# bartelvdh/Navtex

Measured on NVIDIA B200. Metric: iq_msamples_per_s, higher is better.
Workload: dtype f32

## Files before the change

navtex_b200/csrc/demod.cu:

```cuda
#include "demod.cuh"

#include <math.h>
#include <stdlib.h>

namespace nvx {

namespace {

constexpr int kThreads = 128;
constexpr int kPer = 3;
constexpr int kTile = kThreads * kPer;

enum { DS_INIT = 0, DS_WAIT = 1, DS_PENDING = 2 };
enum { BY_WAIT = 1, BY_GOT_DX = 2, BY_GOT_RX = 3 };

__constant__ unsigned char c_ltrs[128];
__constant__ unsigned char c_figs[128];
__constant__ float c_tone_r[5];
__constant__ float c_tone_i[5];
__constant__ double c_tone_rd[5];
__constant__ double c_tone_id[5];

struct Emit {
    uint8_t* ev; int* ev_n; int ev_cap; int n;
    bool writer;
    const unsigned char *ltrs, *figs;
// ... 74 lines not shown
__device__ __forceinline__ void fsm_bit_phasing(FsmState& s, bool is_y) {
    if (s.holdoff != 0) { s.holdoff--; return; }
    constexpr unsigned kYmask = (0xFu << 6) | (0x3u << 12) | (0xFu << 20) | (0x3u << 26);
    if (s.match == 29) {
        if (!is_y) { s.enabled = 1; s.nbits = 0; s.shift = 0; s.holdoff = 1100; }
        s.match = 0;
    } else if ((((kYmask >> s.match) & 1u) != 0) == is_y) {
        s.match++;
    } else if (s.match != 6) {
        s.match = 0;
    }
}


__device__ __forceinline__ size_t pitch_y(int p_max) { return (size_t)kHistY + p_max; }
__device__ __forceinline__ size_t pitch_c(int p_max) { return (size_t)kHistC + p_max + kPadC; }
__host__ __device__ __forceinline__ size_t pitch_p(int p_max) { return ((size_t)p_max / kSpb + 2 + 15) & ~(size_t)15; }
__host__ __device__ __forceinline__ size_t pitch_b(int p_max) { return ((size_t)p_max / (kSpb - 1) + 2 + 15) & ~(size_t)15; }

__device__ __forceinline__ double angle_of(float2 cur, float2 prev) {
    const double yi = cur.x, yq = cur.y, pi = prev.x, pq = prev.y;
    const double re = __dadd_rn(__dmul_rn(yi, pi), __dmul_rn(yq, pq));
    const double im = __dsub_rn(__dmul_rn(yq, pi), __dmul_rn(yi, pq));
    return atan2(im, re);
}

__global__ void __launch_bounds__(kThreads) angle_corr_kernel(const DemodArgs a) {
    __shared__ double s_ang[kTile + 8];
    const int ch = blockIdx.y, tile0 = blockIdx.x * kTile, t = threadIdx.x;
    float2* ybuf = a.b.y3 + (size_t)ch * pitch_y(a.b.p_max);
    const float2* y = ybuf + kHistY;
    if (blockIdx.x == 0) {
        const float2* yp = a.y3_prev + (size_t)ch * pitch_y(a.b.p_max) + a.n_prev;
        if (t < kHistY) ybuf[t] = yp[t];
        double* c = a.b.corr + (size_t)ch * pitch_c(a.b.p_max);
        const double* cp = a.corr_prev + (size_t)ch * pitch_c(a.b.p_max) + a.n_prev;
        for (int k = t; k < kHistC; k += kThreads) c[k] = cp[k];
        __syncthreads();
    }
#pragma unroll
    for (int u = 0; u < kPer; ++u) {
        const int m = tile0 + t + u * kThreads;
        if (m < a.n_new) s_ang[8 + t + u * kThreads] = angle_of(y[m], y[m - 1]);
    }
    if (t < 8) s_ang[t] = angle_of(y[tile0 - 8 + t], y[tile0 - 9 + t]);
    __syncthreads();
    double* corr = a.b.corr + (size_t)ch * pitch_c(a.b.p_max) + kHistC;
#pragma unroll
    for (int u = 0; u < kPer; ++u) {
        const int i = t + u * kThreads, m = tile0 + i;
        if (m >= a.n_new) break;
        double c = s_ang[i + 1];
        c = __dadd_rn(c, s_ang[i + 2]);
        c = __dadd_rn(c, s_ang[i + 3]);
        c = __dsub_rn(c, s_ang[i + 5]);
        c = __dsub_rn(c, s_ang[i + 6]);
        c = __dsub_rn(c, s_ang[i + 7]);
        corr[m] = fabs(c);
    }
}

__device__ __forceinline__ bool window_is_y(const float2* __restrict__ y, float* sums) {
    double br = 0.0, bi = 0.0, yr = 0.0, yi = 0.0;
#pragma unroll
    for (int k = 0; k < 5; ++k) {
        const float srf = y[k].x;
        const double si = (double)y[k].y;
        const float fr = c_tone_r[k], fi = c_tone_i[k];
        const double pr = (double)__fmul_rn(srf, fr), pim = (double)__fmul_rn(srf, fi);
        const double qi = __dmul_rn(si, c_tone_id[k]), qr = __dmul_rn(si, c_tone_rd[k]);
        yr = (double)(float)__dadd_rn(yr, __dsub_rn(pr, qi));
        yi = (double)(float)__dadd_rn(yi, __dadd_rn(pim, qr));
        br = (double)(float)__dadd_rn(br, __dadd_rn(pr, qi));
        bi = (double)(float)__dadd_rn(bi, __dsub_rn(qr, pim));
    }
    const float brf = (float)br, bif = (float)bi, yrf = (float)yr, yif = (float)yi;
    if (sums) { sums[0] = brf; sums[1] = bif; sums[2] = yrf; sums[3] = yif; }
    const float eb = __fadd_rn(__fmul_rn(brf, brf), __fmul_rn(bif, bif));
    const float ey = __fadd_rn(__fmul_rn(yrf, yrf), __fmul_rn(yif, yif));
    return !(eb > ey);
}

constexpr int kSumWarps = 4;
constexpr int kGroup = 7;
__global__ void __launch_bounds__(kSumWarps * 32) offset_sum_kernel(const DemodArgs a, int k_lo, int n_rev) {
    __shared__ double s_os[kSumWarps][3][kGroup][kSpb];
    const int warp = threadIdx.x >> 5, lane = threadIdx.x & 31;
    const int kk = lane / kSpb, j = lane - kk * kSpb;
    const long long unit = ((long long)blockIdx.x * kSumWarps + warp) * 3 + kk;
    const bool mine = kk < 3 && unit < (long long)a.channels * n_rev;
    const int ch = mine ? (int)(unit / n_rev) : 0;
    const int K = k_lo + (mine ? (int)(unit % n_rev) : 0);
    const int m_first = (int)(16 + (long long)kCorrLen * K + j - a.seen);
    const double* cur = a.b.corr + (size_t)ch * pitch_c(a.b.p_max) + kHistC + (m_first - 8);
    const double* prev = cur - kCorrLen;
    const int kk2 = lane / kGroup, u2 = lane - kk2 * kGroup;
    const long long unit2 = ((long long)blockIdx.x * kSumWarps + warp) * 3 + kk2;
    const bool judge = kk2 < 3 && unit2 < (long long)a.channels * n_rev;
    const int ch2 = judge ? (int)(unit2 / n_rev) : 0;
    const int w_first = (int)(24 + (long long)kCorrLen * (k_lo + (judge ? (int)(unit2 % n_rev) : 0)) - a.seen);
    uint8_t* picks2 = a.b.picks + (size_t)ch2 * pitch_p(a.b.p_max);

    double run = 0.0;
#pragma unroll 1
    for (int g = 0; g < kCorrLen / kSpb / kGroup; ++g) {
        const int r0 = g * kGroup;
        const int m0 = m_first + kSpb * r0;
        double acc[kGroup];
        if (mine && m0 < a.n_new) {
#pragma unroll
            for (int u = 0; u < kGroup; ++u) {
                run = __dadd_rn(run, __ldg(cur + kSpb * (r0 + u)));
                acc[u] = run;
            }
        } else {
#pragma unroll
            for (int u = 0; u < kGroup; ++u) acc[u] = 0.0;
        }
        if (mine && m0 < a.n_new && m0 + kSpb * (kGroup - 1) >= -8) {
            const double* p = prev + kSpb * (r0 + 1);
            double v[kGroup - 1];
#pragma unroll
            for (int t = 0; t < kGroup - 1; ++t) v[t] = __ldg(p + kSpb * t);
#pragma unroll
            for (int u = 0; u < kGroup - 1; ++u) {
#pragma unroll
                for (int t = u; t < kGroup - 1; ++t) acc[u] = __dadd_rn(acc[u], v[t]);
            }
            p += kSpb * (kGroup - 1);
            const int rest = kCorrLen / kSpb - kGroup - r0;
#pragma unroll 1
            for (int i = 0; i < rest; i += kGroup, p += kSpb * kGroup) {
                double x[kGroup];
#pragma unroll
                for (int t = 0; t < kGroup; ++t) x[t] = __ldg(p + kSpb * t);
#pragma unroll
                for (int t = 0; t < kGroup; ++t) {
#pragma unroll
                    for (int u = 0; u < kGroup; ++u) acc[u] = __dadd_rn(acc[u], x[t]);
                }
            }
        }
        if (kk < 3) {
#pragma unroll
            for (int u = 0; u < kGroup; ++u) {
                const int m = m0 + kSpb * u;
                const bool ok = mine && m < a.n_new && a.seen + m >= kCorrLen + 7;
                s_os[warp][kk][u][j] = ok ? acc[u] : 0.0;
            }
        }
        __syncwarp();
        if (judge) {
            const int w = w_first + kSpb * (r0 + u2);
            if (w >= 0 && w < a.n_new && a.seen + w >= kCorrLen + 15) {
                double best = -1.0;
                int pick = 0;
#pragma unroll
                for (int i = 0; i < kSpb; ++i) {
                    const double x = s_os[warp][kk2][u2][i];
                    if (x > best) { best = x; pick = i; }
                }
                picks2[w / kSpb] = (uint8_t)pick;
            }
        }
        __syncwarp();
    }
}

constexpr int kSeqWarps = 16;
constexpr int kSeqChunk = 256;
constexpr int kSeqPitch = kSeqChunk + 4;
constexpr int kSeqSmem = kSeqWarps * 32 * kSeqPitch;

__device__ __forceinline__ void stage_rows(uint8_t* s_rows, const uint8_t* src, size_t pitch, int ch0, int channels,
                                           int c0, int count, int lane) {
    __syncwarp();
    const int words = (count + 3) >> 2;
    for (int r = 0; r < 32 && ch0 + r < channels; ++r) {
        const uint32_t* g = reinterpret_cast<const uint32_t*>(src + (size_t)(ch0 + r) * pitch + c0);
        uint32_t* d = reinterpret_cast<uint32_t*>(s_rows + r * kSeqPitch);
// ... 155 lines not shown

__global__ void init_state_kernel(ClockState* clock, FsmState* fsm, int channels) {
    const int ch = blockIdx.x * blockDim.x + threadIdx.x;
    if (ch >= channels) return;
    ClockState c = {};
    c.last_pick = -1;
    c.dstate = DS_INIT;
    clock[ch] = c;
    FsmState s = {};
    s.byte_state = BY_WAIT;
    fsm[ch] = s;
}

}

int demod_launches_per_block() { return 5; }
size_t demod_pick_pitch(int p_max) { return pitch_p(p_max); }
size_t demod_bit_pitch(int p_max) { return pitch_b(p_max); }
int demod_reserved_sms(int channels) {
    const int ctas = (channels + kSeqWarps * 32 - 1) / (kSeqWarps * 32);
    return ctas < 4 ? ctas : 4;
}

cudaError_t demod_init_state(const DemodBuffers& b, int channels, cudaStream_t stream) {
    {
        static const struct { unsigned char code; char l, f; } codes[] = {
            {0x07, 'p', 'p'}, {0x0b, 'J', 'b'}, {0x0d, 'W', '2'}, {0x0e, 'A', '-'}, {0x13, 'F', '*'},
            {0x15, 'Y', '6'}, {0x16, 'S', '\''}, {0x19, '-', '-'}, {0x1a, 'D', '%'}, {0x1c, 'Z', '+'},
            {0x1d, '_', ' '}, {0x23, 'C', ':'}, {0x25, 'P', '0'}, {0x26, 'I', '8'}, {0x29, 'G', '*'},
            {0x2a, 'R', '4'}, {0x2c, 'L', ')'}, {0x31, 'M', '.'}, {0x32, 'N', ','}, {0x34, 'H', '*'},
            {0x38, 'O', '9'}, {0x43, 'K', '('}, {0x45, 'Q', '1'}, {0x46, 'U', '7'}, {0x49, 'f', 'f'},
// ... 10 lines not shown
            tr[i] = cosf(ang);
            ti[i] = sinf(ang);
        }
        cudaError_t e;
        if ((e = cudaMemcpyToSymbol(c_ltrs, ltrs, sizeof ltrs)) != cudaSuccess) return e;
        if ((e = cudaMemcpyToSymbol(c_figs, figs, sizeof figs)) != cudaSuccess) return e;
        if ((e = cudaMemcpyToSymbol(c_tone_r, tr, sizeof tr)) != cudaSuccess) return e;
        if ((e = cudaMemcpyToSymbol(c_tone_i, ti, sizeof ti)) != cudaSuccess) return e;
        double trd[5], tid[5];
        for (int i = 0; i < 5; ++i) { trd[i] = tr[i]; tid[i] = ti[i]; }
        if ((e = cudaMemcpyToSymbol(c_tone_rd, trd, sizeof trd)) != cudaSuccess) return e;
        if ((e = cudaMemcpyToSymbol(c_tone_id, tid, sizeof tid)) != cudaSuccess) return e;
    }
    cudaError_t e;
    if ((e = cudaMemsetAsync(b.y3, 0, sizeof(float2) * (size_t)channels * (kHistY + b.p_max), stream)) != cudaSuccess) return e;
    if ((e = cudaMemsetAsync(b.corr, 0, sizeof(double) * (size_t)channels * (kHistC + b.p_max + kPadC), stream)) != cudaSuccess) return e;
    if ((e = cudaMemsetAsync(b.picks, 0, (size_t)channels * pitch_p(b.p_max), stream)) != cudaSuccess) return e;
    init_state_kernel<<<(channels + 127) / 128, 128, 0, stream>>>(b.clock, b.fsm, channels);
    return cudaGetLastError();
}

cudaError_t demod_launch(const DemodArgs& a, cudaStream_t s_ff, cudaStream_t s_seq, cudaEvent_t ff_done, cudaEvent_t* marks) {
    if (a.n_new <= 0 || a.channels <= 0) return cudaSuccess;
    auto mark = [&](int k, cudaStream_t st) { if (marks) cudaEventRecord(marks[k], st); };
    mark(0, s_ff);
    angle_corr_kernel<<<dim3((a.n_new + kTile - 1) / kTile, a.channels), kThreads, 0, s_ff>>>(a);
    mark(1, s_ff);
    {
        const long long lo = a.seen - 8 - (kCorrLen + 15), hi = a.seen + a.n_new - 17;
        const int k_lo = lo <= 0 ? 0 : (int)((lo + kCorrLen - 1) / kCorrLen);
        if (hi >= 0 && (int)(hi / kCorrLen) >= k_lo) {
            const int n_rev = (int)(hi / kCorrLen) - k_lo + 1;
            const long long units = (long long)a.channels * n_rev;
            offset_sum_kernel<<<(unsigned)((units + 3 * kSumWarps - 1) / (3 * kSumWarps)), kSumWarps * 32, 0, s_ff>>>(a, k_lo, n_rev);
        }
    }
    mark(2, s_ff);
    mark(3, s_ff);
    {
        cudaError_t e = cudaEventRecord(ff_done, s_ff);
        if (e != cudaSuccess) return e;
        if (s_seq != s_ff && (e = cudaStreamWaitEvent(s_seq, ff_done, 0)) != cudaSuccess) return e;
    }
    {
        cudaError_t e = cudaFuncSetAttribute(symbol_clock_kernel, cudaFuncAttributeMaxDynamicSharedMemorySize, kSeqSmem);
        if (e == cudaSuccess) e = cudaFuncSetAttribute(fsm_kernel, cudaFuncAttributeMaxDynamicSharedMemorySize, kSeqSmem);
        if (e != cudaSuccess) return e;
    }
    const unsigned seq_ctas = (a.channels + kSeqWarps * 32 - 1) / (kSeqWarps * 32);
    mark(4, s_seq);
// ... 11 lines not shown
```

navtex_b200/csrc/demod.cuh:

```cuda
#pragma once
#include <cuda_runtime.h>
#include <stdint.h>

namespace nvx {

constexpr int kSpb = 9;
constexpr int kCorrLen = 63 * kSpb;
constexpr int kEvAbort = 0x18;

constexpr int kHistY = 16;
constexpr int kHistC = 640;
constexpr int kPadC = 64;

struct ClockState {
    int last_pick;
    int dstate, offs, next_offs, cur, pend;
};

struct FsmState {
    int match;
    int byte_state, figures, nbits, shift;
    unsigned dx_ring;
    int dx_at, dx_full;
    unsigned err_mask;
    int err_at, err_full, err_count;
    int eoe_count, prev_dx_alpha, holdoff, enabled;
};

struct DemodBuffers {
    float2* y3;
    double* corr;
    uint8_t* picks;
    int* bitpos;
    uint8_t* bitval;
    int* nbits;
    ClockState* clock;
    FsmState* fsm;
    int p_max;
};

struct DemodArgs {
    DemodBuffers b;
    const float2* y3_prev;
    const double* corr_prev;
    int n_prev;
    int n_new;
    int channels;
    long long seen;
    uint8_t* events;
    int* ev_count;
    int ev_cap;
    char* bits;
    float* disc;
    int* bit_count;
    int bit_cap;
};

size_t demod_pick_pitch(int p_max);
size_t demod_bit_pitch(int p_max);
int demod_reserved_sms(int channels);
cudaError_t demod_launch(const DemodArgs& a, cudaStream_t s_ff, cudaStream_t s_seq, cudaEvent_t ff_done, cudaEvent_t* marks = nullptr);
cudaError_t demod_init_state(const DemodBuffers& b, int channels, cudaStream_t stream);
int demod_launches_per_block();

}
```

navtex_b200/csrc/engine.cu:

```cuda
#include <cuda.h>
#include <cuda_runtime.h>
#include <math.h>
#include <stdarg.h>
#include <stdio.h>
#include <stdlib.h>
#include <string.h>

#include <condition_variable>
#include <mutex>
#include <string>
#include <thread>
#include <vector>

#include "../../include/navtex_b200.h"
#include "demod.cuh"
#include "fir_cascade.cuh"
#include "fir_long.cuh"
#include "message_assembler.h"

namespace nvx {
int cascade_box_elems(SampleFmt f);
int cascade_tap_class(int n1, int n2, int n3);
int cascade_warm_super(int tap_class);
void cascade_fill_taps(int tap_class, const double* h1, int n1, const double* h2, int n2, const double* h3, int n3, CascadeTaps* out);
// ... 70 lines not shown
    const unsigned w[4] = {(unsigned)v.x, (unsigned)v.y, (unsigned)v.z, (unsigned)v.w};
    int o[8];
#pragma unroll
    for (int k = 0; k < 4; ++k) {
        o[2 * k] = (int)(((w[k] & 0xFFu) - 128u) & 0xFFFFu) | (int)(((((w[k] >> 8) & 0xFFu) - 128u) & 0xFFFFu) << 16);
        o[2 * k + 1] = (int)((((w[k] >> 16) & 0xFFu) - 128u) & 0xFFFFu) | (int)((((w[k] >> 24) - 128u) & 0xFFFFu) << 16);
    }
    int4* dst = reinterpret_cast<int4*>(out + i);
    dst[0] = make_int4(o[0], o[1], o[2], o[3]);
    dst[1] = make_int4(o[4], o[5], o[6], o[7]);
}

}

constexpr int kBuf = 3;

struct nvx_engine {
    nvx_config cfg;
    int S = 0, P_max = 0, channels = 0;
    int C = 2;
    cudaStream_t stream = nullptr;
    cudaStream_t stream_demod = nullptr;
    float2* y3buf[kBuf] = {};
    uint8_t* pickbuf[kBuf] = {};
    cudaEvent_t casc_done[kBuf] = {}, demod_done[kBuf] = {}, ff_done[kBuf] = {};
    long long blocks = 0;
    int last_buf = 0;
    int tap_class = 0;
    int halo = 1960;
    void* tail[nvx::kSampleFmts][2] = {};
    CUtensorMap map_tail[nvx::kSampleFmts][2];
    int tail_cur = 0;
    int fmt = -1;
    short2* u8_wide = nullptr;
    nvx::DemodBuffers db = {};
    double* corrbuf[2] = {nullptr, nullptr};
    uint8_t* d_events[kBuf] = {}; int* d_ev_count[kBuf] = {}; int ev_cap = 0;
    char* d_bits = nullptr; float* d_disc = nullptr; int* d_bit_count = nullptr; int bit_cap = 0;
    uint8_t* h_events[kBuf] = {}; int* h_ev_count[kBuf] = {};
    cudaStream_t stream_copy = nullptr;
    void* stage[2] = {nullptr, nullptr};
    size_t stage_bytes[2] = {0, 0};
    cudaEvent_t copy_done[2] = {}, stage_free[2] = {};
    long long host_pushes = 0;
    long long sb_abs = 0;
    int last_P = 0;
    bool custom_taps = false;
    nvx::CascadeTaps taps;
    nvx::NcoParam* d_nco = nullptr;
    nvx::NcoChan* d_nco_ch = nullptr;
    bool long_taps = false;
    nvx::LongStage lst[3];
    float2* lhist[3][2] = {};
    float2 *y1buf = nullptr, *y2buf = nullptr;
    int lcur = 0;
    nvx::LongTcStage* ltc[2] = {nullptr, nullptr};
    bool mix_on_load = false;
    bool ltc_wanted[2] = {false, false};
    nvx::LongStageTaps ltaps[3];
    std::vector<int> stream_tag;
    bool serial = false;
    bool ff_on_main = true;
    int target_warps[nvx::kSampleFmts] = {576, 576, 576};
    nvx::MessageAssembler assembler;
    std::vector<nvx::AssembledMessage> ready, handed;
    std::vector<nvx_message> view;
    nvx_message_cb cb = nullptr; void* cb_user = nullptr;
    std::thread worker;
    std::mutex mu;
    std::condition_variable cv;
    long long queued = 0, drained = 0;
    long long delivered = 0;
    bool stop = false;
    int worker_rc = 0;
    int timing = 0;
    std::vector<cudaEvent_t> ev_pool;
    struct Span { int a, b, kind; };
    std::vector<Span> spans;
    size_t ev_used = 0;
    std::vector<float> cascade_spans_ms;
    nvx_stats stats = {};
};

namespace {

int free_engine(nvx_engine* e) {
    if (!e) return 0;
    cudaSetDevice(e->cfg.device);
    if (e->stream) cudaStreamSynchronize(e->stream);
    if (e->stream_demod) cudaStreamSynchronize(e->stream_demod);
    if (e->worker.joinable()) {
        {
            std::lock_guard<std::mutex> lk(e->mu);
            e->stop = true;
        }
        e->cv.notify_all();
        e->worker.join();
    }
    for (cudaEvent_t ev : e->ev_pool) cudaEventDestroy(ev);
    for (int f = 0; f < nvx::kSampleFmts; ++f) { cudaFree(e->tail[f][0]); cudaFree(e->tail[f][1]); }
    cudaFree(e->u8_wide);
    cudaFree(e->corrbuf[0]); cudaFree(e->corrbuf[1]); cudaFree(e->db.clock); cudaFree(e->db.fsm);
    cudaFree(e->db.bitpos); cudaFree(e->db.bitval); cudaFree(e->db.nbits);
    cudaFree(e->d_bits); cudaFree(e->d_disc); cudaFree(e->d_bit_count);
    if (e->stream_copy) cudaStreamSynchronize(e->stream_copy);
    for (int k = 0; k < 2; ++k) {
        cudaFree(e->stage[k]);
        if (e->copy_done[k]) cudaEventDestroy(e->copy_done[k]);
        if (e->stage_free[k]) cudaEventDestroy(e->stage_free[k]);
    }
    if (e->stream_copy) cudaStreamDestroy(e->stream_copy);
    cudaFree(e->d_nco);
    cudaFree(e->d_nco_ch);
    for (int k = 0; k < 3; ++k) { cudaFree(e->lhist[k][0]); cudaFree(e->lhist[k][1]); }
    cudaFree(e->y1buf); cudaFree(e->y2buf);
    nvx::long_tc_free(e->ltc[0]); nvx::long_tc_free(e->ltc[1]);
    for (int k = 0; k < kBuf; ++k) {
        cudaFree(e->y3buf[k]); cudaFree(e->d_events[k]); cudaFree(e->d_ev_count[k]);
        cudaFreeHost(e->h_events[k]); cudaFreeHost(e->h_ev_count[k]);
        if (e->casc_done[k]) cudaEventDestroy(e->casc_done[k]);
        if (e->demod_done[k]) cudaEventDestroy(e->demod_done[k]);
        if (e->ff_done[k]) cudaEventDestroy(e->ff_done[k]);
        cudaFree(e->pickbuf[k]);
    }
    if (e->stream) cudaStreamDestroy(e->stream);
    if (e->stream_demod) cudaStreamDestroy(e->stream_demod);
    delete e;
    return 0;
}

int reset_state(nvx_engine* e) {
    for (int f = 0; f < nvx::kSampleFmts; ++f)
        for (int k = 0; k < 2; ++k)
            CU_TRY(cudaMemsetAsync(e->tail[f][k], (nvx::SampleFmt)f == nvx::SampleFmt::U8 ? 128 : 0,
                                   (size_t)e->S * e->halo * nvx::sample_bytes((nvx::SampleFmt)f), e->stream));
    e->fmt = -1;
    if (e->long_taps)
        for (int k = 0; k < 3; ++k)
            for (int q = 0; q < 2; ++q)
                CU_TRY(cudaMemsetAsync(e->lhist[k][q], 0, (size_t)(k == 0 ? e->S : e->channels) * e->lst[k].H * sizeof(float2), e->stream));
    e->lcur = 0;
    for (int k = 0; k < kBuf; ++k) {
        e->db.y3 = e->y3buf[k];
        e->db.picks = e->pickbuf[k];
        e->db.corr = e->corrbuf[k & 1];
        CU_TRY(nvx::demod_init_state(e->db, e->channels, e->stream));
    }
    CU_TRY(cudaStreamSynchronize(e->stream));
    e->tail_cur = 0;
    e->sb_abs = 0;
    e->last_P = 0;
    e->blocks = 0;
    e->last_buf = 0;
    {
        std::lock_guard<std::mutex> lk(e->mu);
        e->queued = e->drained = 0;
        e->worker_rc = 0;
    }
    e->assembler.reset();
    e->ready.clear();
// ... 161 lines not shown
    ca.nco = e->d_nco_ch;
    ca.y3_pitch = nvx::kHistY + e->P_max;
    ca.y3_off = nvx::kHistY;
    ca.ch_total = e->C;
    ca.ch0 = 0;

    if (!e->ff_on_main && e->blocks >= 2) CU_TRY(cudaStreamWaitEvent(e->stream, e->ff_done[(b + 1) % kBuf], 0));
    cudaEvent_t t0 = nullptr, t1 = nullptr, marks[8] = {};
    if (e->timing) {
        const int base = (int)e->ev_used;
        t0 = next_event(e); t1 = next_event(e);
        e->spans.push_back({base, base + 1, 0});
        if (e->timing > 1) {
            for (int k = 0; k < 8; ++k) marks[k] = next_event(e);
            e->spans.push_back({base + 2, base + 9, 1});
            for (int k = 0; k < 3; ++k) e->spans.push_back({base + 2 + k, base + 3 + k, 2 + k});
            for (int k = 0; k < 3; ++k) e->spans.push_back({base + 6 + k, base + 7 + k, 5 + k});
        }
        CU_TRY(cudaEventRecord(t0, e->stream));
    }
    if (e->long_taps) {
        if (fmt == SampleFmt::U8) {
            if (!e->u8_wide) CU_TRY(cudaMalloc(&e->u8_wide, (size_t)e->S * e->cfg.max_block * sizeof(short2)));
            const long long count = (long long)e->S * n;
            widen_u8_kernel<<<(unsigned)((count / 8 + 255) / 256), 256, 0, e->stream>>>(static_cast<const uchar2*>(d_x), e->u8_wide, count);
            CU_TRY(cudaGetLastError());
            e->stats.aux_launches++;
            d_x = e->u8_wide;
        }
        const int s16 = fmt != SampleFmt::F32;
        const int cur = e->lcur, nx = cur ^ 1;
// ... 55 lines not shown
            tail_carry_kernel<short2><<<grid, 256, 0, e->stream>>>(static_cast<const short2*>(old_tail), static_cast<const short2*>(d_x),
                                                                   static_cast<short2*>(new_tail), e->S, n, e->halo);
        else
            tail_carry_kernel<float2><<<grid, 256, 0, e->stream>>>(static_cast<const float2*>(old_tail), static_cast<const float2*>(d_x),
                                                                   static_cast<float2*>(new_tail), e->S, n, e->halo);
        CU_TRY(cudaGetLastError());
    }
    e->tail_cur = nxt;

    CU_TRY(cudaEventRecord(e->casc_done[b], e->stream));

    DemodArgs da;
    da.b = e->db;
    da.b.y3 = e->y3buf[b];
    da.b.picks = e->pickbuf[b];
    da.b.corr = e->corrbuf[e->blocks & 1];
    da.y3_prev = e->y3buf[(b + kBuf - 1) % kBuf];
    da.corr_prev = e->corrbuf[(e->blocks & 1) ^ 1];
    da.n_prev = e->last_P;
    da.n_new = n_super; da.channels = e->channels; da.seen = e->sb_abs;
    da.events = e->d_events[b]; da.ev_count = e->d_ev_count[b]; da.ev_cap = e->ev_cap;
    da.bits = e->d_bits; da.disc = e->d_disc; da.bit_count = e->d_bit_count; da.bit_cap = e->bit_cap;
    cudaStream_t s_ff = e->ff_on_main ? e->stream : e->stream_demod;
    if (!e->ff_on_main) CU_TRY(cudaStreamWaitEvent(e->stream_demod, e->casc_done[b], 0));
    CU_TRY(demod_launch(da, s_ff, e->stream_demod, e->ff_done[b], e->timing > 1 ? marks : nullptr));
    CU_TRY(cudaMemcpyAsync(e->h_ev_count[b], e->d_ev_count[b], sizeof(int) * e->channels, cudaMemcpyDeviceToHost, e->stream_demod));
    CU_TRY(cudaMemcpyAsync(e->h_events[b], e->d_events[b], (size_t)e->channels * e->ev_cap, cudaMemcpyDeviceToHost, e->stream_demod));
    CU_TRY(cudaEventRecord(e->demod_done[b], e->stream_demod));
    if (e->serial) CU_TRY(cudaStreamWaitEvent(e->stream, e->demod_done[b], 0));
    e->last_buf = b;
    e->blocks++;
    {
        std::lock_guard<std::mutex> lk(e->mu);
        e->queued = e->blocks;
    }
    e->cv.notify_all();
    e->sb_abs += n_super;
    e->last_P = n_super;
    e->stats.cascade_launches++;
    e->stats.demod_launches += nvx::demod_launches_per_block();
// ... 104 lines not shown
        const int D[3] = {NVX_D1, NVX_D2, NVX_D3};
        for (int k = 0; k < 3; ++k) e->lst[k] = nvx::long_stage(D[k], n[k]);
    }
    e->ev_cap = 2 * (e->P_max / 63 + 2) + 8;
    e->bit_cap = cfg->keep_bits ? e->P_max / 8 + 2 : 0;
#define CREATE_TRY(expr)                                                                                      \
    do {                                                                                                      \
        cudaError_t e__ = (expr);                                                                             \
        if (e__ != cudaSuccess) {                                                                             \
            fail(NVX_ERR_CUDA, "%s failed: %s", #expr, cudaGetErrorString(e__));                              \
            free_engine(e);                                                                                   \
            return e__ == cudaErrorMemoryAllocation ? NVX_ERR_NOMEM : NVX_ERR_CUDA;                           \
        }                                                                                                     \
    } while (0)
    {
        int lo = 0, hi = 0;
        CREATE_TRY(cudaDeviceGetStreamPriorityRange(&lo, &hi));
        CREATE_TRY(cudaStreamCreateWithPriority(&e->stream, cudaStreamNonBlocking, lo));
        CREATE_TRY(cudaStreamCreateWithFlags(&e->stream_copy, cudaStreamNonBlocking));
        for (int k = 0; k < 2; ++k) {
            CREATE_TRY(cudaEventCreateWithFlags(&e->copy_done[k], cudaEventDisableTiming));
            CREATE_TRY(cudaEventCreateWithFlags(&e->stage_free[k], cudaEventDisableTiming));
        }
        CREATE_TRY(cudaStreamCreateWithPriority(&e->stream_demod, cudaStreamNonBlocking, hi));
        const char* mode = getenv("NVX_PIPELINE");
        e->serial = mode && !strcmp(mode, "serial");
        e->ff_on_main = !(mode && !strcmp(mode, "overlap"));
    }
    for (int k = 0; k < kBuf; ++k) {
        CREATE_TRY(cudaEventCreateWithFlags(&e->casc_done[k], cudaEventDisableTiming));
        CREATE_TRY(cudaEventCreateWithFlags(&e->demod_done[k], cudaEventDisableTiming));
        CREATE_TRY(cudaEventCreateWithFlags(&e->ff_done[k], cudaEventDisableTiming));
    }
    for (int f = 0; f < nvx::kSampleFmts; ++f)
        for (int k = 0; k < 2; ++k)
            CREATE_TRY(cudaMalloc(&e->tail[f][k], (size_t)e->S * e->halo * nvx::sample_bytes((nvx::SampleFmt)f)));
    e->db.p_max = e->P_max;
    for (int k = 0; k < kBuf; ++k) CREATE_TRY(cudaMalloc(&e->y3buf[k], (size_t)e->channels * (nvx::kHistY + e->P_max) * sizeof(float2)));
    for (int k = 0; k < 2; ++k) CREATE_TRY(cudaMalloc(&e->corrbuf[k], (size_t)e->channels * (nvx::kHistC + e->P_max + nvx::kPadC) * sizeof(double)));
    for (int k = 0; k < kBuf; ++k) CREATE_TRY(cudaMalloc(&e->pickbuf[k], (size_t)e->channels * nvx::demod_pick_pitch(e->P_max)));
    CREATE_TRY(cudaMalloc(&e->db.bitpos, (size_t)e->channels * nvx::demod_bit_pitch(e->P_max) * sizeof(int)));
    CREATE_TRY(cudaMalloc(&e->db.bitval, (size_t)e->channels * nvx::demod_bit_pitch(e->P_max)));
    CREATE_TRY(cudaMalloc(&e->db.nbits, (size_t)e->channels * sizeof(int)));
    CREATE_TRY(cudaMemset(e->db.nbits, 0, (size_t)e->channels * sizeof(int)));
    CREATE_TRY(cudaMalloc(&e->db.clock, (size_t)e->channels * sizeof(nvx::ClockState)));
    CREATE_TRY(cudaMalloc(&e->db.fsm, (size_t)e->channels * sizeof(nvx::FsmState)));
    for (int k = 0; k < kBuf; ++k) {
        CREATE_TRY(cudaMalloc(&e->d_events[k], (size_t)e->channels * e->ev_cap));
        CREATE_TRY(cudaMalloc(&e->d_ev_count[k], sizeof(int) * e->channels));
        CREATE_TRY(cudaMemset(e->d_ev_count[k], 0, sizeof(int) * e->channels));
        CREATE_TRY(cudaMallocHost(&e->h_events[k], (size_t)e->channels * e->ev_cap));
        CREATE_TRY(cudaMallocHost(&e->h_ev_count[k], sizeof(int) * e->channels));
        memset(e->h_ev_count[k], 0, sizeof(int) * e->channels);
    }
// ... 27 lines not shown
        nvx::cascade_fill_taps(e->tap_class, cfg->h1, n[0], cfg->h2, n[1], cfg->h3, n[2], &e->taps);
    }
    if (!nco.empty()) {
        CREATE_TRY(cudaMalloc(&e->d_nco, nco.size() * sizeof(nvx::NcoParam)));
        CREATE_TRY(cudaMemcpy(e->d_nco, nco.data(), nco.size() * sizeof(nvx::NcoParam), cudaMemcpyHostToDevice));
    }
    if (!nco_ch.empty()) {
        CREATE_TRY(cudaMalloc(&e->d_nco_ch, nco_ch.size() * sizeof(nvx::NcoChan)));
        CREATE_TRY(cudaMemcpy(e->d_nco_ch, nco_ch.data(), nco_ch.size() * sizeof(nvx::NcoChan), cudaMemcpyHostToDevice));
    }
#undef CREATE_TRY
    for (int f = 0; f < nvx::kSampleFmts; ++f)
        for (int k = 0; k < 2; ++k)
            if (int rc = encode_rows(&e->map_tail[f][k], e->tail[f][k], e->halo, e->S, (nvx::SampleFmt)f)) { free_engine(e); return rc; }
    for (int f = 0; f < nvx::kSampleFmts; ++f)
        e->target_warps[f] = nvx::cascade_target_warps(cfg->device, nvx::demod_reserved_sms(e->channels), (nvx::SampleFmt)f, e->tap_class, C > 2);
    e->assembler.resize(e->channels);
    if (int rc = reset_state(e)) { free_engine(e); return rc; }
    e->worker = std::thread(worker_main, e);
    *out = e;
    return 0;
}

void nvx_engine_destroy(nvx_engine* e) { free_engine(e); }

int nvx_engine_reset(nvx_engine* e) {
    if (!e) return fail(NVX_ERR_ARG, "null engine");
    CU_TRY(cudaSetDevice(e->cfg.device));
    const int rc_sync = sync_engine(e);
    if (rc_sync == NVX_ERR_CUDA) return rc_sync;
    {
// ... 238 lines not shown
```

Measured before the change: 694,500.

## Fuse angle correlation and offset sum into one per-channel shared-memory kernel

Replaces the angle_corr and offset_sum kernels with a single persistent bitsync_ff_kernel. Each block owns a channel and computes the correlation into a sliding shared-memory window instead of a full global corr buffer, keeping only a small history buffer between blocks. This removes one launch per block and the global round trip of the double-precision correlation array. It also adds optional confinement of the kernel to a few SMs on a separate stream, off by default. The trade-off is reduced parallelism: one block per channel with chunked serial processing, plus a prefix rescan of running sums per item.

```diff
diff --git a/navtex_b200/csrc/demod.cu b/navtex_b200/csrc/demod.cu
--- a/navtex_b200/csrc/demod.cu
+++ b/navtex_b200/csrc/demod.cu
@@ -7,9 +7,7 @@
 
 namespace {
 
-constexpr int kThreads = 128;
 constexpr int kPer = 3;
-constexpr int kTile = kThreads * kPer;
 
 enum { DS_INIT = 0, DS_WAIT = 1, DS_PENDING = 2 };
 enum { BY_WAIT = 1, BY_GOT_DX = 2, BY_GOT_RX = 3 };
@@ -114,7 +112,6 @@
 
 
 __device__ __forceinline__ size_t pitch_y(int p_max) { return (size_t)kHistY + p_max; }
-__device__ __forceinline__ size_t pitch_c(int p_max) { return (size_t)kHistC + p_max + kPadC; }
 __host__ __device__ __forceinline__ size_t pitch_p(int p_max) { return ((size_t)p_max / kSpb + 2 + 15) & ~(size_t)15; }
 __host__ __device__ __forceinline__ size_t pitch_b(int p_max) { return ((size_t)p_max / (kSpb - 1) + 2 + 15) & ~(size_t)15; }
 
@@ -123,41 +120,6 @@
     const double re = __dadd_rn(__dmul_rn(yi, pi), __dmul_rn(yq, pq));
     const double im = __dsub_rn(__dmul_rn(yq, pi), __dmul_rn(yi, pq));
     return atan2(im, re);
-}
-
-__global__ void __launch_bounds__(kThreads) angle_corr_kernel(const DemodArgs a) {
-    __shared__ double s_ang[kTile + 8];
-    const int ch = blockIdx.y, tile0 = blockIdx.x * kTile, t = threadIdx.x;
-    float2* ybuf = a.b.y3 + (size_t)ch * pitch_y(a.b.p_max);
-    const float2* y = ybuf + kHistY;
-    if (blockIdx.x == 0) {
-        const float2* yp = a.y3_prev + (size_t)ch * pitch_y(a.b.p_max) + a.n_prev;
-        if (t < kHistY) ybuf[t] = yp[t];
-        double* c = a.b.corr + (size_t)ch * pitch_c(a.b.p_max);
-        const double* cp = a.corr_prev + (size_t)ch * pitch_c(a.b.p_max) + a.n_prev;
-        for (int k = t; k < kHistC; k += kThreads) c[k] = cp[k];
-        __syncthreads();
-    }
-#pragma unroll
-    for (int u = 0; u < kPer; ++u) {
-        const int m = tile0 + t + u * kThreads;
-        if (m < a.n_new) s_ang[8 + t + u * kThreads] = angle_of(y[m], y[m - 1]);
-    }
-    if (t < 8) s_ang[t] = angle_of(y[tile0 - 8 + t], y[tile0 - 9 + t]);
-    __syncthreads();
-    double* corr = a.b.corr + (size_t)ch * pitch_c(a.b.p_max) + kHistC;
-#pragma unroll
-    for (int u = 0; u < kPer; ++u) {
-        const int i = t + u * kThreads, m = tile0 + i;
-        if (m >= a.n_new) break;
-        double c = s_ang[i + 1];
-        c = __dadd_rn(c, s_ang[i + 2]);
-        c = __dadd_rn(c, s_ang[i + 3]);
-        c = __dsub_rn(c, s_ang[i + 5]);
-        c = __dsub_rn(c, s_ang[i + 6]);
-        c = __dsub_rn(c, s_ang[i + 7]);
-        corr[m] = fabs(c);
-    }
 }
 
 __device__ __forceinline__ bool window_is_y(const float2* __restrict__ y, float* sums) {
@@ -181,89 +143,183 @@
     return !(eb > ey);
 }
 
-constexpr int kSumWarps = 4;
 constexpr int kGroup = 7;
-__global__ void __launch_bounds__(kSumWarps * 32) offset_sum_kernel(const DemodArgs a, int k_lo, int n_rev) {
-    __shared__ double s_os[kSumWarps][3][kGroup][kSpb];
-    const int warp = threadIdx.x >> 5, lane = threadIdx.x & 31;
+#ifndef NVX_FF_THREADS
+#define NVX_FF_THREADS 256
+#endif
+constexpr int kFfThreads = NVX_FF_THREADS;
+constexpr int kFfWarps = kFfThreads / 32;
+constexpr int kFfTile = kFfThreads * kPer;
+#ifndef NVX_FF_REV
+#define NVX_FF_REV 6
+#endif
+#ifndef NVX_FF_CTAS
+#define NVX_FF_CTAS 4
+#endif
+constexpr int kFfRev = NVX_FF_REV;
+constexpr int kFfBack = 64 * kSpb;
+constexpr int kFfWin = kFfBack + kCorrLen * kFfRev;
+constexpr int kFfPatch = 3 * kGroup * kSpb;
+constexpr int kFfSmem = (int)sizeof(double) * (kFfWin + (kFfTile + 8 > kFfWarps * kFfPatch ? kFfTile + 8 : kFfWarps * kFfPatch));
+constexpr int kFfCtasPerSm = NVX_FF_CTAS;
+constexpr int kFfSmemAlone = 60 * 1024;
+constexpr int kFfCtasAlone = 3;
+static_assert(kCorrLen * kFfRev >= kFfBack, "the window front is moved in one pass");
+static_assert(kFfRev % 3 == 0, "a warp item covers three revolutions");
+
+__global__ void __launch_bounds__(kFfThreads, kFfCtasPerSm) bitsync_ff_kernel(const DemodArgs a, int k_lo, int n_rev, int n_chunks) {
+    extern __shared__ __align__(16) double s_ff[];
+    double* const sc = s_ff;
+    double* const s_ang = sc + kFfWin;
+    const int t = threadIdx.x, warp = t >> 5, lane = t & 31;
+    double* const s_os = sc + kFfWin + warp * kFfPatch;
+    const int n_new = a.n_new;
+    const long long seen = a.seen;
+    const int s0 = (int)(16 + (long long)kCorrLen * k_lo - seen);
     const int kk = lane / kSpb, j = lane - kk * kSpb;
-    const long long unit = ((long long)blockIdx.x * kSumWarps + warp) * 3 + kk;
-    const bool mine = kk < 3 && unit < (long long)a.channels * n_rev;
-    const int ch = mine ? (int)(unit / n_rev) : 0;
-    const int K = k_lo + (mine ? (int)(unit % n_rev) : 0);
-    const int m_first = (int)(16 + (long long)kCorrLen * K + j - a.seen);
-    const double* cur = a.b.corr + (size_t)ch * pitch_c(a.b.p_max) + kHistC + (m_first - 8);
-    const double* prev = cur - kCorrLen;
     const int kk2 = lane / kGroup, u2 = lane - kk2 * kGroup;
-    const long long unit2 = ((long long)blockIdx.x * kSumWarps + warp) * 3 + kk2;
-    const bool judge = kk2 < 3 && unit2 < (long long)a.channels * n_rev;
-    const int ch2 = judge ? (int)(unit2 / n_rev) : 0;
-    const int w_first = (int)(24 + (long long)kCorrLen * (k_lo + (judge ? (int)(unit2 % n_rev) : 0)) - a.seen);
-    uint8_t* picks2 = a.b.picks + (size_t)ch2 * pitch_p(a.b.p_max);
-
-    double run = 0.0;
+
+    for (int ch = blockIdx.x; ch < a.channels; ch += gridDim.x) {
+        float2* ybuf = a.b.y3 + (size_t)ch * pitch_y(a.b.p_max);
+        const float2* y = ybuf + kHistY;
+        const double* h_old = a.hist_prev + (size_t)ch * kHistC;
+        double* h_new = a.b.hist + (size_t)ch * kHistC;
+        uint8_t* picks = a.b.picks + (size_t)ch * pitch_p(a.b.p_max);
+        if (t < kHistY) ybuf[t] = a.y3_prev[(size_t)ch * pitch_y(a.b.p_max) + a.n_prev + t];
+        for (int k = t; k + n_new < kHistC; k += kFfThreads) h_new[k] = h_old[k + n_new];
+        {
+            const int base = s0 - kFfBack;
+            for (int i = t; base + i < 0; i += kFfThreads) sc[i] = base + i >= -kHistC ? h_old[base + i + kHistC] : 0.0;
+        }
+        double front = t < 8 ? angle_of(y[t - 8], y[t - 9]) : 0.0;
+        __syncthreads();
+
+        for (int c = 0; c < n_chunks; ++c) {
+            const int base = s0 - kFfBack + kCorrLen * kFfRev * c;
+            if (c > 0) {
+                for (int i = t; i < kFfBack; i += kFfThreads) sc[i] = sc[i + kCorrLen * kFfRev];
+                __syncthreads();
+            }
+            const int lo = c == 0 ? 0 : base + kFfBack, end = base + kFfWin, hi = min(end, n_new);
+            for (int m = max(lo, n_new) + t; m < end; m += kFfThreads) sc[m - base] = 0.0;
+            float2 ya[kPer], yb[kPer];
+            auto load = [&](int t0) {
+#pragma unroll
+                for (int u = 0; u < kPer; ++u) {
+                    const int m = t0 + t + u * kFfThreads;
+                    if (m < hi) { ya[u] = y[m]; yb[u] = y[m - 1]; }
+                }
+            };
+            if (lo < hi) load(lo);
+            for (int t0 = lo; t0 < hi; t0 += kFfTile) {
+                if (t < 8) s_ang[t] = front;
+                float2 ca[kPer], cb[kPer];
+#pragma unroll
+                for (int u = 0; u < kPer; ++u) { ca[u] = ya[u]; cb[u] = yb[u]; }
+                if (t0 + kFfTile < hi) load(t0 + kFfTile);
+#pragma unroll
+                for (int u = 0; u < kPer; ++u) {
+                    const int i = t + u * kFfThreads, m = t0 + i;
+                    if (m < hi) s_ang[8 + i] = angle_of(ca[u], cb[u]);
+                }
+                __syncthreads();
+                if (t < 8) front = s_ang[min(hi - t0, kFfTile) + t];
+#pragma unroll
+                for (int u = 0; u < kPer; ++u) {
+                    const int i = t + u * kFfThreads, m = t0 + i;
+                    if (m >= hi) break;
+                    double v = s_ang[i + 1];
+                    v = __dadd_rn(v, s_ang[i + 2]);
+                    v = __dadd_rn(v, s_ang[i + 3]);
+                    v = __dsub_rn(v, s_ang[i + 5]);
+                    v = __dsub_rn(v, s_ang[i + 6]);
+                    v = __dsub_rn(v, s_ang[i + 7]);
+                    v = fabs(v);
+                    sc[m - base] = v;
+                    if (m >= n_new - kHistC) h_new[m - (n_new - kHistC)] = v;
+                }
+                __syncthreads();
+            }
+            __syncthreads();
+
 #pragma unroll 1
-    for (int g = 0; g < kCorrLen / kSpb / kGroup; ++g) {
-        const int r0 = g * kGroup;
-        const int m0 = m_first + kSpb * r0;
-        double acc[kGroup];
-        if (mine && m0 < a.n_new) {
-#pragma unroll
-            for (int u = 0; u < kGroup; ++u) {
-                run = __dadd_rn(run, __ldg(cur + kSpb * (r0 + u)));
-                acc[u] = run;
-            }
-        } else {
-#pragma unroll
-            for (int u = 0; u < kGroup; ++u) acc[u] = 0.0;
-        }
-        if (mine && m0 < a.n_new && m0 + kSpb * (kGroup - 1) >= -8) {
-            const double* p = prev + kSpb * (r0 + 1);
-            double v[kGroup - 1];
-#pragma unroll
-            for (int t = 0; t < kGroup - 1; ++t) v[t] = __ldg(p + kSpb * t);
-#pragma unroll
-            for (int u = 0; u < kGroup - 1; ++u) {
-#pragma unroll
-                for (int t = u; t < kGroup - 1; ++t) acc[u] = __dadd_rn(acc[u], v[t]);
-            }
-            p += kSpb * (kGroup - 1);
-            const int rest = kCorrLen / kSpb - kGroup - r0;
+            for (int q = 0;; ++q) {
+                const int item = q * kFfWarps + ((q & 1) ? kFfWarps - 1 - warp : warp);
+                if (item >= kFfRev / 3 * (kCorrLen / kSpb / kGroup)) break;
+                const int g = item / (kFfRev / 3), p = item - kFfRev / 3 * g;
+                const int r0 = g * kGroup;
+                const int k_rel = kFfRev * c + 3 * p;
+                if (k_rel >= n_rev) continue;
+                const bool mine = kk < 3 && k_rel + kk < n_rev;
+                const int kr = mine ? 3 * p + kk : 0;
+                const int m_first = base + kFfBack + kCorrLen * kr + j;
+                const int m0 = m_first + kSpb * r0;
+                const double* cur = sc + (kFfBack - 8 + kCorrLen * kr + j);
+                const double* prev = cur - kCorrLen;
+                double acc[kGroup];
+                if (mine && m0 < n_new) {
+                    double run = 0.0;
 #pragma unroll 1
-            for (int i = 0; i < rest; i += kGroup, p += kSpb * kGroup) {
-                double x[kGroup];
-#pragma unroll
-                for (int t = 0; t < kGroup; ++t) x[t] = __ldg(p + kSpb * t);
-#pragma unroll
-                for (int t = 0; t < kGroup; ++t) {
-#pragma unroll
-                    for (int u = 0; u < kGroup; ++u) acc[u] = __dadd_rn(acc[u], x[t]);
-                }
-            }
-        }
-        if (kk < 3) {
-#pragma unroll
-            for (int u = 0; u < kGroup; ++u) {
-                const int m = m0 + kSpb * u;
-                const bool ok = mine && m < a.n_new && a.seen + m >= kCorrLen + 7;
-                s_os[warp][kk][u][j] = ok ? acc[u] : 0.0;
-            }
-        }
-        __syncwarp();
-        if (judge) {
-            const int w = w_first + kSpb * (r0 + u2);
-            if (w >= 0 && w < a.n_new && a.seen + w >= kCorrLen + 15) {
-                double best = -1.0;
-                int pick = 0;
-#pragma unroll
-                for (int i = 0; i < kSpb; ++i) {
-                    const double x = s_os[warp][kk2][u2][i];
-                    if (x > best) { best = x; pick = i; }
-                }
-                picks2[w / kSpb] = (uint8_t)pick;
-            }
-        }
-        __syncwarp();
+                    for (int r = 0; r < r0; ++r) run = __dadd_rn(run, cur[kSpb * r]);
+#pragma unroll
+                    for (int u = 0; u < kGroup; ++u) {
+                        run = __dadd_rn(run, cur[kSpb * (r0 + u)]);
+                        acc[u] = run;
+                    }
+                } else {
+#pragma unroll
+                    for (int u = 0; u < kGroup; ++u) acc[u] = 0.0;
+                }
+                if (mine && m0 < n_new && m0 + kSpb * (kGroup - 1) >= -8) {
+                    const double* pp = prev + kSpb * (r0 + 1);
+                    double v[kGroup - 1];
+#pragma unroll
+                    for (int s = 0; s < kGroup - 1; ++s) v[s] = pp[kSpb * s];
+#pragma unroll
+                    for (int u = 0; u < kGroup - 1; ++u) {
+#pragma unroll
+                        for (int s = u; s < kGroup - 1; ++s) acc[u] = __dadd_rn(acc[u], v[s]);
+                    }
+                    pp += kSpb * (kGroup - 1);
+                    const int rest = kCorrLen / kSpb - kGroup - r0;
+#pragma unroll 1
+                    for (int i = 0; i < rest; i += kGroup, pp += kSpb * kGroup) {
+                        double x[kGroup];
+#pragma unroll
+                        for (int s = 0; s < kGroup; ++s) x[s] = pp[kSpb * s];
+#pragma unroll
+                        for (int s = 0; s < kGroup; ++s) {
+#pragma unroll
+                            for (int u = 0; u < kGroup; ++u) acc[u] = __dadd_rn(acc[u], x[s]);
+                        }
+                    }
+                }
+                if (kk < 3) {
+#pragma unroll
+                    for (int u = 0; u < kGroup; ++u) {
+                        const int m = m0 + kSpb * u;
+                        const bool ok = mine && m < n_new && seen + m >= kCorrLen + 7;
+                        s_os[(kk * kGroup + u) * kSpb + j] = ok ? acc[u] : 0.0;
+                    }
+                }
+                __syncwarp();
+                if (kk2 < 3 && k_rel + kk2 < n_rev) {
+                    const int w = base + kFfBack + kCorrLen * (3 * p + kk2) + 8 + kSpb * (r0 + u2);
+                    if (w >= 0 && w < n_new && seen + w >= kCorrLen + 15) {
+                        double best = -1.0;
+                        int pick = 0;
+#pragma unroll
+                        for (int i = 0; i < kSpb; ++i) {
+                            const double x = s_os[(kk2 * kGroup + u2) * kSpb + i];
+                            if (x > best) { best = x; pick = i; }
+                        }
+                        picks[w / kSpb] = (uint8_t)pick;
+                    }
+                }
+                __syncwarp();
+            }
+            __syncthreads();
+        }
     }
 }
 
@@ -449,7 +505,8 @@
 
 }
 
-int demod_launches_per_block() { return 5; }
+int demod_launches_per_block() { return 4; }
+int demod_ff_ctas_per_sm() { return kFfCtasAlone; }
 size_t demod_pick_pitch(int p_max) { return pitch_p(p_max); }
 size_t demod_bit_pitch(int p_max) { return pitch_b(p_max); }
 int demod_reserved_sms(int channels) {
@@ -490,26 +547,27 @@
     }
     cudaError_t e;
     if ((e = cudaMemsetAsync(b.y3, 0, sizeof(float2) * (size_t)channels * (kHistY + b.p_max), stream)) != cudaSuccess) return e;
-    if ((e = cudaMemsetAsync(b.corr, 0, sizeof(double) * (size_t)channels * (kHistC + b.p_max + kPadC), stream)) != cudaSuccess) return e;
+    if ((e = cudaMemsetAsync(b.hist, 0, sizeof(double) * (size_t)channels * kHistC, stream)) != cudaSuccess) return e;
     if ((e = cudaMemsetAsync(b.picks, 0, (size_t)channels * pitch_p(b.p_max), stream)) != cudaSuccess) return e;
     init_state_kernel<<<(channels + 127) / 128, 128, 0, stream>>>(b.clock, b.fsm, channels);
     return cudaGetLastError();
 }
 
-cudaError_t demod_launch(const DemodArgs& a, cudaStream_t s_ff, cudaStream_t s_seq, cudaEvent_t ff_done, cudaEvent_t* marks) {
+cudaError_t demod_launch(const DemodArgs& a, cudaStream_t s_ff, cudaStream_t s_seq, cudaEvent_t ff_done, cudaEvent_t* marks, int ff_ctas) {
     if (a.n_new <= 0 || a.channels <= 0) return cudaSuccess;
     auto mark = [&](int k, cudaStream_t st) { if (marks) cudaEventRecord(marks[k], st); };
-    mark(0, s_ff);
-    angle_corr_kernel<<<dim3((a.n_new + kTile - 1) / kTile, a.channels), kThreads, 0, s_ff>>>(a);
-    mark(1, s_ff);
     {
         const long long lo = a.seen - 8 - (kCorrLen + 15), hi = a.seen + a.n_new - 17;
         const int k_lo = lo <= 0 ? 0 : (int)((lo + kCorrLen - 1) / kCorrLen);
-        if (hi >= 0 && (int)(hi / kCorrLen) >= k_lo) {
-            const int n_rev = (int)(hi / kCorrLen) - k_lo + 1;
-            const long long units = (long long)a.channels * n_rev;
-            offset_sum_kernel<<<(unsigned)((units + 3 * kSumWarps - 1) / (3 * kSumWarps)), kSumWarps * 32, 0, s_ff>>>(a, k_lo, n_rev);
-        }
+        const int n_rev = hi >= 0 && (int)(hi / kCorrLen) >= k_lo ? (int)(hi / kCorrLen) - k_lo + 1 : 0;
+        const int n_chunks = n_rev > 0 ? (n_rev + kFfRev - 1) / kFfRev : 1;
+        const int smem = ff_ctas > 0 ? (kFfSmem > kFfSmemAlone ? kFfSmem : kFfSmemAlone) : kFfSmem;
+        cudaError_t e = cudaFuncSetAttribute(bitsync_ff_kernel, cudaFuncAttributeMaxDynamicSharedMemorySize, smem);
+        if (e != cudaSuccess) return e;
+        const unsigned grid = (unsigned)(ff_ctas > 0 && ff_ctas < a.channels ? ff_ctas : a.channels);
+        mark(0, s_ff);
+        bitsync_ff_kernel<<<grid, kFfThreads, smem, s_ff>>>(a, k_lo, n_rev, n_chunks);
+        mark(1, s_ff);
     }
     mark(2, s_ff);
     mark(3, s_ff);
diff --git a/navtex_b200/csrc/demod.cuh b/navtex_b200/csrc/demod.cuh
--- a/navtex_b200/csrc/demod.cuh
+++ b/navtex_b200/csrc/demod.cuh
@@ -10,7 +10,6 @@
 
 constexpr int kHistY = 16;
 constexpr int kHistC = 640;
-constexpr int kPadC = 64;
 
 struct ClockState {
     int last_pick;
@@ -29,7 +28,7 @@
 
 struct DemodBuffers {
     float2* y3;
-    double* corr;
+    double* hist;
     uint8_t* picks;
     int* bitpos;
     uint8_t* bitval;
@@ -42,7 +41,7 @@
 struct DemodArgs {
     DemodBuffers b;
     const float2* y3_prev;
-    const double* corr_prev;
+    const double* hist_prev;
     int n_prev;
     int n_new;
     int channels;
@@ -59,7 +58,9 @@
 size_t demod_pick_pitch(int p_max);
 size_t demod_bit_pitch(int p_max);
 int demod_reserved_sms(int channels);
-cudaError_t demod_launch(const DemodArgs& a, cudaStream_t s_ff, cudaStream_t s_seq, cudaEvent_t ff_done, cudaEvent_t* marks = nullptr);
+cudaError_t demod_launch(const DemodArgs& a, cudaStream_t s_ff, cudaStream_t s_seq, cudaEvent_t ff_done, cudaEvent_t* marks = nullptr,
+                         int ff_ctas = 0);
+int demod_ff_ctas_per_sm();
 cudaError_t demod_init_state(const DemodBuffers& b, int channels, cudaStream_t stream);
 int demod_launches_per_block();
 
diff --git a/navtex_b200/csrc/engine.cu b/navtex_b200/csrc/engine.cu
--- a/navtex_b200/csrc/engine.cu
+++ b/navtex_b200/csrc/engine.cu
@@ -108,6 +108,10 @@
 }
 
 constexpr int kBuf = 3;
+#ifndef NVX_FF_SMS_DEFAULT
+#define NVX_FF_SMS_DEFAULT 0
+#endif
+constexpr int kFfSmsDefault = NVX_FF_SMS_DEFAULT;
 
 struct nvx_engine {
     nvx_config cfg;
@@ -115,6 +119,7 @@
     int C = 2;
     cudaStream_t stream = nullptr;
     cudaStream_t stream_demod = nullptr;
+    cudaStream_t stream_ff = nullptr;
     float2* y3buf[kBuf] = {};
     uint8_t* pickbuf[kBuf] = {};
     cudaEvent_t casc_done[kBuf] = {}, demod_done[kBuf] = {}, ff_done[kBuf] = {};
@@ -128,7 +133,7 @@
     int fmt = -1;
     short2* u8_wide = nullptr;
     nvx::DemodBuffers db = {};
-    double* corrbuf[2] = {nullptr, nullptr};
+    double* histbuf[2] = {nullptr, nullptr};
     uint8_t* d_events[kBuf] = {}; int* d_ev_count[kBuf] = {}; int ev_cap = 0;
     char* d_bits = nullptr; float* d_disc = nullptr; int* d_bit_count = nullptr; int bit_cap = 0;
     uint8_t* h_events[kBuf] = {}; int* h_ev_count[kBuf] = {};
@@ -155,6 +160,7 @@
     std::vector<int> stream_tag;
     bool serial = false;
     bool ff_on_main = true;
+    int ff_sms = 0;
     int target_warps[nvx::kSampleFmts] = {576, 576, 576};
     nvx::MessageAssembler assembler;
     std::vector<nvx::AssembledMessage> ready, handed;
@@ -183,6 +189,7 @@
     cudaSetDevice(e->cfg.device);
     if (e->stream) cudaStreamSynchronize(e->stream);
     if (e->stream_demod) cudaStreamSynchronize(e->stream_demod);
+    if (e->stream_ff) cudaStreamSynchronize(e->stream_ff);
     if (e->worker.joinable()) {
         {
             std::lock_guard<std::mutex> lk(e->mu);
@@ -194,7 +201,7 @@
     for (cudaEvent_t ev : e->ev_pool) cudaEventDestroy(ev);
     for (int f = 0; f < nvx::kSampleFmts; ++f) { cudaFree(e->tail[f][0]); cudaFree(e->tail[f][1]); }
     cudaFree(e->u8_wide);
-    cudaFree(e->corrbuf[0]); cudaFree(e->corrbuf[1]); cudaFree(e->db.clock); cudaFree(e->db.fsm);
+    cudaFree(e->histbuf[0]); cudaFree(e->histbuf[1]); cudaFree(e->db.clock); cudaFree(e->db.fsm);
     cudaFree(e->db.bitpos); cudaFree(e->db.bitval); cudaFree(e->db.nbits);
     cudaFree(e->d_bits); cudaFree(e->d_disc); cudaFree(e->d_bit_count);
     if (e->stream_copy) cudaStreamSynchronize(e->stream_copy);
@@ -219,6 +226,7 @@
     }
     if (e->stream) cudaStreamDestroy(e->stream);
     if (e->stream_demod) cudaStreamDestroy(e->stream_demod);
+    if (e->stream_ff) cudaStreamDestroy(e->stream_ff);
     delete e;
     return 0;
 }
@@ -237,7 +245,7 @@
     for (int k = 0; k < kBuf; ++k) {
         e->db.y3 = e->y3buf[k];
         e->db.picks = e->pickbuf[k];
-        e->db.corr = e->corrbuf[k & 1];
+        e->db.hist = e->histbuf[k & 1];
         CU_TRY(nvx::demod_init_state(e->db, e->channels, e->stream));
     }
     CU_TRY(cudaStreamSynchronize(e->stream));
@@ -429,7 +437,7 @@
         if (e->timing > 1) {
             for (int k = 0; k < 8; ++k) marks[k] = next_event(e);
             e->spans.push_back({base + 2, base + 9, 1});
-            for (int k = 0; k < 3; ++k) e->spans.push_back({base + 2 + k, base + 3 + k, 2 + k});
+            e->spans.push_back({base + 2, base + 3, 2});
             for (int k = 0; k < 3; ++k) e->spans.push_back({base + 6 + k, base + 7 + k, 5 + k});
         }
         CU_TRY(cudaEventRecord(t0, e->stream));
@@ -515,16 +523,16 @@
     da.b = e->db;
     da.b.y3 = e->y3buf[b];
     da.b.picks = e->pickbuf[b];
-    da.b.corr = e->corrbuf[e->blocks & 1];
+    da.b.hist = e->histbuf[e->blocks & 1];
     da.y3_prev = e->y3buf[(b + kBuf - 1) % kBuf];
-    da.corr_prev = e->corrbuf[(e->blocks & 1) ^ 1];
+    da.hist_prev = e->histbuf[(e->blocks & 1) ^ 1];
     da.n_prev = e->last_P;
     da.n_new = n_super; da.channels = e->channels; da.seen = e->sb_abs;
     da.events = e->d_events[b]; da.ev_count = e->d_ev_count[b]; da.ev_cap = e->ev_cap;
     da.bits = e->d_bits; da.disc = e->d_disc; da.bit_count = e->d_bit_count; da.bit_cap = e->bit_cap;
-    cudaStream_t s_ff = e->ff_on_main ? e->stream : e->stream_demod;
-    if (!e->ff_on_main) CU_TRY(cudaStreamWaitEvent(e->stream_demod, e->casc_done[b], 0));
-    CU_TRY(demod_launch(da, s_ff, e->stream_demod, e->ff_done[b], e->timing > 1 ? marks : nullptr));
+    cudaStream_t s_ff = e->ff_on_main ? e->stream : e->stream_ff ? e->stream_ff : e->stream_demod;
+    if (!e->ff_on_main) CU_TRY(cudaStreamWaitEvent(s_ff, e->casc_done[b], 0));
+    CU_TRY(demod_launch(da, s_ff, e->stream_demod, e->ff_done[b], e->timing > 1 ? marks : nullptr, e->ff_sms * nvx::demod_ff_ctas_per_sm()));
     CU_TRY(cudaMemcpyAsync(e->h_ev_count[b], e->d_ev_count[b], sizeof(int) * e->channels, cudaMemcpyDeviceToHost, e->stream_demod));
     CU_TRY(cudaMemcpyAsync(e->h_events[b], e->d_events[b], (size_t)e->channels * e->ev_cap, cudaMemcpyDeviceToHost, e->stream_demod));
     CU_TRY(cudaEventRecord(e->demod_done[b], e->stream_demod));
@@ -659,18 +667,23 @@
         }                                                                                                     \
     } while (0)
     {
+        const char* mode = getenv("NVX_PIPELINE");
+        e->serial = mode && !strcmp(mode, "serial");
+        e->ff_on_main = !(mode && !strcmp(mode, "overlap"));
+        e->ff_sms = getenv("NVX_FF_SMS") ? atoi(getenv("NVX_FF_SMS")) : (mode ? 0 : kFfSmsDefault);
+        if (e->ff_sms < 0 || e->ff_sms > 64) e->ff_sms = 0;
+        if (e->ff_sms) e->ff_on_main = false;
         int lo = 0, hi = 0;
         CREATE_TRY(cudaDeviceGetStreamPriorityRange(&lo, &hi));
-        CREATE_TRY(cudaStreamCreateWithPriority(&e->stream, cudaStreamNonBlocking, lo));
+        const int main_prio = e->ff_sms && hi < lo ? lo - 1 : lo;
+        CREATE_TRY(cudaStreamCreateWithPriority(&e->stream, cudaStreamNonBlocking, main_prio));
+        if (e->ff_sms) CREATE_TRY(cudaStreamCreateWithPriority(&e->stream_ff, cudaStreamNonBlocking, lo));
         CREATE_TRY(cudaStreamCreateWithFlags(&e->stream_copy, cudaStreamNonBlocking));
         for (int k = 0; k < 2; ++k) {
             CREATE_TRY(cudaEventCreateWithFlags(&e->copy_done[k], cudaEventDisableTiming));
             CREATE_TRY(cudaEventCreateWithFlags(&e->stage_free[k], cudaEventDisableTiming));
         }
         CREATE_TRY(cudaStreamCreateWithPriority(&e->stream_demod, cudaStreamNonBlocking, hi));
-        const char* mode = getenv("NVX_PIPELINE");
-        e->serial = mode && !strcmp(mode, "serial");
-        e->ff_on_main = !(mode && !strcmp(mode, "overlap"));
     }
     for (int k = 0; k < kBuf; ++k) {
         CREATE_TRY(cudaEventCreateWithFlags(&e->casc_done[k], cudaEventDisableTiming));
@@ -682,7 +695,7 @@
             CREATE_TRY(cudaMalloc(&e->tail[f][k], (size_t)e->S * e->halo * nvx::sample_bytes((nvx::SampleFmt)f)));
     e->db.p_max = e->P_max;
     for (int k = 0; k < kBuf; ++k) CREATE_TRY(cudaMalloc(&e->y3buf[k], (size_t)e->channels * (nvx::kHistY + e->P_max) * sizeof(float2)));
-    for (int k = 0; k < 2; ++k) CREATE_TRY(cudaMalloc(&e->corrbuf[k], (size_t)e->channels * (nvx::kHistC + e->P_max + nvx::kPadC) * sizeof(double)));
+    for (int k = 0; k < 2; ++k) CREATE_TRY(cudaMalloc(&e->histbuf[k], (size_t)e->channels * nvx::kHistC * sizeof(double)));
     for (int k = 0; k < kBuf; ++k) CREATE_TRY(cudaMalloc(&e->pickbuf[k], (size_t)e->channels * nvx::demod_pick_pitch(e->P_max)));
     CREATE_TRY(cudaMalloc(&e->db.bitpos, (size_t)e->channels * nvx::demod_bit_pitch(e->P_max) * sizeof(int)));
     CREATE_TRY(cudaMalloc(&e->db.bitval, (size_t)e->channels * nvx::demod_bit_pitch(e->P_max)));
@@ -740,7 +753,7 @@
         for (int k = 0; k < 2; ++k)
             if (int rc = encode_rows(&e->map_tail[f][k], e->tail[f][k], e->halo, e->S, (nvx::SampleFmt)f)) { free_engine(e); return rc; }
     for (int f = 0; f < nvx::kSampleFmts; ++f)
-        e->target_warps[f] = nvx::cascade_target_warps(cfg->device, nvx::demod_reserved_sms(e->channels), (nvx::SampleFmt)f, e->tap_class, C > 2);
+        e->target_warps[f] = nvx::cascade_target_warps(cfg->device, nvx::demod_reserved_sms(e->channels) + e->ff_sms, (nvx::SampleFmt)f, e->tap_class, C > 2);
     e->assembler.resize(e->channels);
     if (int rc = reset_state(e)) { free_engine(e); return rc; }
     e->worker = std::thread(worker_main, e);
```

Result: no change. 695,200, median of 6 (+0.1%).
